# kuboyoo/alphazero-general-ori

Hardware: AMD Instinct MI355X
Metric: self-play rollouts/sec (32k boards, 2p Splendor) at 1/2/4/8 MI355X (higher is better)
Workload: dtype fp32 (network) / int8 (boards) / f64 (tree statistics)

## Files before the change

alphazero-general-ori_amd/csrc/mcts.hip:

```cpp
#include <hip/hip_runtime.h>

#include <cmath>
#include <cstring>
#include <new>

#include "../../include/splendor_amd.h"

#include "mcts_device.h"

using namespace spl;

#ifndef SPL_BOUNDS_CHECK
#define SPL_BOUNDS_CHECK 0
#endif
#if SPL_BOUNDS_CHECK
__device__ unsigned long long g_bounds[4 + 64];
__device__ __noinline__ void bounds_note(int site, long long v, int t) {
    atomicAdd(&g_bounds[4 + (site & 63)], 1ull);
    if (atomicAdd(&g_bounds[0], 1ull) == 0) {
        g_bounds[1] = (unsigned long long)v; g_bounds[2] = (unsigned long long)site; g_bounds[3] = (unsigned long long)t;
    }
}
#define BCHK(cond, site, v, t, fix)                                   \
    do {                                                               \
// ... 1730 lines not shown
    }
#endif
}

#ifndef LM_PROBE
#define LM_PROBE 0
#endif
#if LM_PROBE
constexpr int LM_PSLOTS = 4096;
__device__ unsigned long long g_lm_probe[LM_PSLOTS][8];
#define LMPROBE(k) \
    if (threadIdx.x == 0 && blockIdx.x < LM_PSLOTS) g_lm_probe[blockIdx.x][k] = __builtin_amdgcn_s_memrealtime();
#else
#define LMPROBE(k)
#endif
template <int N>
__global__ __launch_bounds__(256) void k_leaf_mask(Pools P, int B, int lim, const int8_t *__restrict__ leaf_state,
                                                   const uint8_t *__restrict__ leaf_valid,
                                                   uint64_t *__restrict__ leaf_mask,
                                                   int32_t *__restrict__ leaf_index,
                                                   int32_t *__restrict__ leaf_count) {
    using Lx = Lay<N>;
    using Cv = Conv<N>;
    constexpr int RB = 64, ST = (Lx::ROWS % 2 ? Lx::ROWS : Lx::ROWS + 1) * 8;
    __shared__ __align__(16) int8_t lds[RB * ST];
    __shared__ uint64_t mfac[7 * 116];
    __shared__ uint64_t pf0[4][RB], pf1[RB];
    __shared__ uint32_t pcond[RB];
    __shared__ uint8_t pbad[4][RB];
    __shared__ uint64_t msk[RB][7];
    LMPROBE(0)
    const int b0 = blockIdx.x * RB, nb = min(RB, B - b0);
    const int tid = threadIdx.x, w = tid >> 6, l = lane_id();
    if (w == 2 && leaf_index) {
        const bool v = l < nb && leaf_valid[b0 + l];
        const uint64_t bv = __ballot(v);
        if (v) leaf_index[b0 + __popcll(bv & lanemask_lt())] = b0 + l;
        if (l == 0) leaf_count[blockIdx.x] = __popcll(bv);
    }
    constexpr int FW = (7 * 116 + 255) / 256;
    uint64_t fw[FW];
#pragma unroll
    for (int k = 0; k < FW; k++) {
        const int i = tid + 256 * k;
        fw[k] = i < 7 * 116 ? (&K_MASK_FACTORS[0][0])[i] : 0;
    }
    if constexpr (Cv::QUAD) {
        constexpr int BU = (RB * Cv::UNITS + 255) / 256;
        uint32_t d[BU][7];
#pragma unroll
        for (int k = 0; k < BU; k++) {
            const int i = min(tid + 256 * k, nb * Cv::UNITS - 1), b = i / Cv::UNITS, u = i - b * Cv::UNITS;
            const uint32_t *g = reinterpret_cast<const uint32_t *>(leaf_state + (size_t)(b0 + b) * Lx::S) + 7 * u;
#pragma unroll
// ... 1 lines not shown
        }
#pragma unroll
        for (int k = 0; k < BU; k++) {
            const int i = tid + 256 * k, b = i / Cv::UNITS, u = i - b * Cv::UNITS;
            if (i < nb * Cv::UNITS) quad_rows_put(d[k], reinterpret_cast<uint64_t *>(lds + b * ST) + 4 * u);
        }
    } else {
        for (int i = tid; i < nb * Cv::UNITS; i += 256) {
            const int b = i / Cv::UNITS, u = i - b * Cv::UNITS;
            Cv::load(lds + b * ST, leaf_state + (size_t)(b0 + b) * Lx::S, u);
        }
    }
#pragma unroll
    for (int k = 0; k < FW; k++)
        if (tid + 256 * k < 7 * 116) mfac[tid + 256 * k] = fw[k];
    lds_sync();
    LMPROBE(1)
    if (l < nb) {
        uint64_t f0, f1;
        uint32_t cc;
        bool bad;
        const int8_t *st = lds + l * ST;
        switch (w) {
            case 0: lane_predicates_part<N, 0>(st, 0, lim, f0, f1, cc, bad); break;
            case 1: lane_predicates_part<N, 1>(st, 0, lim, f0, f1, cc, bad); break;
            case 2: lane_predicates_part<N, 2>(st, 0, lim, f0, f1, cc, bad); break;
            default: lane_predicates_part<N, 3>(st, 0, lim, f0, f1, cc, bad); break;
        }
        pf0[w][l] = f0;
        if (w == 3) pf1[l] = f1;
        if (w == 2) pcond[l] = cc;
        pbad[w][l] = bad;
// ... 26 lines not shown
        }
    }
    lds_sync();
    LMPROBE(3)
    {
        const int b = 16 * w + l;
        if (l < 16 && b < nb) {
            int cnt = 0;
#pragma unroll
            for (int k = 0; k < 7; k++) cnt += __popcll(msk[b][k]);
            if (!cnt) msk[b][6] |= 1ull << (408 - 384);
        }
    }
    lds_sync();
    LMPROBE(4)
    for (int i = tid; i < nb * 7; i += 256)
        if (leaf_valid[b0 + i / 7]) leaf_mask[(size_t)b0 * 7 + i] = (&msk[0][0])[i];
    LMPROBE(5)
}

#ifndef BK_PF
#define BK_PF 4
#endif
#ifndef BK_WIDE
#define BK_WIDE 12
#endif
#ifndef BACKUP_WAVES
#define BACKUP_WAVES 4
#endif

struct Screen {
    float L1, H1, H2, cf, ff, sqv, sqe;
// ... 1092 lines not shown
}

int spl_mcts_pick_best(spl_mcts *m, const uint8_t *active, uint32_t board_base, uint32_t stream,
                       int16_t *action, void *hs) {
    if (!m || !action || stream > 0xFFFFFFu) return SPL_EINVAL;
    hipLaunchKernelGGL(k_pick_best, wave_grid(m->B), dim3(THREADS), 0, (hipStream_t)hs, m->P, m->cfg,
                       m->B, active, board_base, stream, action);
    return check_launch();
}

static int launch_select(spl_mcts *m, int8_t *leaf_state, uint64_t *leaf_mask, uint8_t *leaf_valid,
                         int32_t *leaf_index, int32_t *leaf_count, void *hs) {
    SPL_DISPATCH(m->n, hipLaunchKernelGGL(k_select_lanes<N>, dim3((unsigned)((m->B + 63) / 64)), dim3(64), 0,
                                          (hipStream_t)hs, m->P, m->cfg, m->B, mcts_lim(m),
                                          leaf_state, leaf_valid));
    SPL_DISPATCH(m->n, hipLaunchKernelGGL(k_leaf_mask<N>, dim3((unsigned)((m->B + 63) / 64)), dim3(256), 0,
                                          (hipStream_t)hs, m->P, m->B, mcts_lim(m), leaf_state, leaf_valid,
                                          leaf_mask, leaf_index, leaf_count));
    return check_launch();
}

int spl_mcts_select(spl_mcts *m, int8_t *leaf_state, uint64_t *leaf_mask, uint8_t *leaf_valid,
                    void *hs) {
    if (!m || !leaf_state || !leaf_mask || !leaf_valid) return SPL_EINVAL;
    return launch_select(m, leaf_state, leaf_mask, leaf_valid, nullptr, nullptr, hs);
}

int spl_mcts_select_compact(spl_mcts *m, int8_t *leaf_state, uint64_t *leaf_mask, uint8_t *leaf_valid,
                            int32_t *leaf_index, int32_t *leaf_count, void *hs) {
    if (!m || !leaf_state || !leaf_mask || !leaf_valid || !leaf_index || !leaf_count) return SPL_EINVAL;
    return launch_select(m, leaf_state, leaf_mask, leaf_valid, leaf_index, leaf_count, hs);
}

int spl_mcts_backup_kind(spl_mcts *m, const uint64_t *leaf_mask, const float *pi, const float *v, int kinds,
// ... 132 lines not shown
```

alphazero-general-ori_amd/csrc/nnet.hip:

```cpp
#include <hip/hip_runtime.h>

#include "../../include/splendor_amd.h"

#ifndef NN_PROBE
#define NN_PROBE 0
#endif
#if NN_PROBE
__device__ unsigned long long g_nn_probe[16];
#define NPROBE(k)                                                  \
    if (threadIdx.x == 0) {                                        \
        const uint64_t c_ = __builtin_readcyclecounter();          \
        atomicAdd(&g_nn_probe[k], (unsigned long long)(c_ - nlast)); \
        nlast = c_;                                                \
    }
#else
#define NPROBE(k)
#endif

namespace {

typedef float f32x16 __attribute__((ext_vector_type(16)));
typedef float f32x4 __attribute__((ext_vector_type(4)));
typedef float f32x2 __attribute__((ext_vector_type(2)));

// ... 59 lines not shown
            s -= nstages(l);
        }
        return -1;
    }
    static constexpr int stg_index(int s) {
        for (int l = 0; l < 4; l++) {
            if (s < nstages(l)) return s;
            s -= nstages(l);
        }
        return -1;
    }
    static constexpr int stg_c0(int s) { return stg_index(s) ? first(stg_layer(s)) : 0; }
    static constexpr int stg_nc(int s) { return stg_index(s) ? CL[stg_layer(s)] - first(stg_layer(s)) : first(stg_layer(s)); }
};
static_assert(Net<4>::XR + RING <= BUFA, "input staging + weight ring fit bufA");

template <int V> struct IntC {
    static constexpr int value = V;
};

typedef __bf16 bf16x8 __attribute__((ext_vector_type(8)));
typedef uint32_t u32x4 __attribute__((ext_vector_type(4)));
struct F8 {
    float4 lo, hi;
};

__device__ __forceinline__ uint32_t hi_pair(uint32_t a, uint32_t b) { return __builtin_amdgcn_perm(b, a, 0x07060302u); }
__device__ __forceinline__ void split8(const F8 &x, bf16x8 &hi, bf16x8 &mid, bf16x8 &lo) {
    const float xs[8] = {x.lo.x, x.lo.y, x.lo.z, x.lo.w, x.hi.x, x.hi.y, x.hi.z, x.hi.w};
    float r1[8], r2[8];
// ... 201 lines not shown
        __builtin_amdgcn_fence(__ATOMIC_RELEASE, "wavefront");
        __builtin_amdgcn_wave_barrier();
        int f = lane < ML ? rowt[lane] : -1;
        f = max(f, __builtin_amdgcn_update_dpp(-1, f, 0x111, 0xf, 0xf, false));
        f = max(f, __builtin_amdgcn_update_dpp(-1, f, 0x112, 0xf, 0xf, false));
        f = max(f, __builtin_amdgcn_update_dpp(-1, f, 0x114, 0xf, 0xf, false));
        f = max(f, __builtin_amdgcn_update_dpp(-1, f, 0x118, 0xf, 0xf, false));
        f = max(f, __builtin_amdgcn_update_dpp(-1, f, 0x142, 0xa, 0xf, false));
        const int pos = f >= 0 ? b0 + lane + offv[f] : 0;
        __builtin_amdgcn_wave_barrier();
        if (lane < ML) rowt[lane] = pos;
    }
    return base;
}

template <int NP, int PR>
__global__ __launch_bounds__(NNT) __attribute__((amdgpu_waves_per_eu(2, 2))) void k_nn_forward(int B, const int8_t *__restrict__ state,
                                                    const uint64_t *__restrict__ mask,
                                                    const float *__restrict__ W, float *__restrict__ pi_out,
                                                    float *__restrict__ v_out,
                                                    const int32_t *__restrict__ idx,
                                                    const int32_t *__restrict__ count) {
    using Nt = Net<NP>;
    constexpr int R = Nt::R, X0S = Nt::X0S, NSTG = Nt::NSTG;
    __shared__ __align__(16) char lds[BUFA + SAB + ML * 7 * 8 + 15 * ML * 4];
    float *bufA = reinterpret_cast<float *>(lds);
    SplitAct *SB0 = reinterpret_cast<SplitAct *>(lds + BUFA);
    uint64_t *mskl = reinterpret_cast<uint64_t *>(lds + BUFA + SAB);
    const int tid = threadIdx.x, w = __builtin_amdgcn_readfirstlane(tid >> 6), lane = tid & 63, li = lane & 31;
    const int h = lane >> 5;
    const int b0 = blockIdx.x * ML;
    const float *aff = W + Nt::AFF;
    char *ring = lds + Nt::XR;
    float *biasL = reinterpret_cast<float *>(SB0);
    auto load_stage = [&](auto s_const) {
        constexpr int S = decltype(s_const)::value;
        if constexpr (S < NSTG) {
            constexpr int L = Nt::stg_layer(S), C0 = Nt::stg_c0(S), NC = Nt::stg_nc(S), C = Nt::CL[L];
            const char *src = reinterpret_cast<const char *>(W + Nt::soff(L)) + lane * 16;
            char *dst = ring + (S & 1) * RSTAGE * RSLOT;
#pragma unroll
            for (int j = 0; j < NC; j++)
#pragma unroll
                for (int b = 0; b < 4; b++)
#pragma unroll
                    for (int p = 0; p < PR; p++)
                        glds16(src + ((b * C + C0 + j) * 3 + p) * 1024, dst + ((j * 4 + b) * 3 + p) * 1024);
        }
    };
    if (w == 7) {
        load_stage(IntC<0>());
        load_stage(IntC<1>());
    }
    int *rowt = reinterpret_cast<int *>(lds + BUFA + SAB + ML * 7 * 8);
    int *rowt_w = rowt + (w < 7 ? w : 0) * ML, *rowv = rowt + 7 * ML, *offv_w = rowt + (8 + (w < 7 ? w : 0)) * ML;
    int cnt = B;
    if (count) {
        cnt = __builtin_amdgcn_readfirstlane(
            nn_list_rows(count, (B + 63) >> 6, b0, w < 7 ? rowt_w : nullptr, offv_w));
        __builtin_amdgcn_fence(__ATOMIC_RELEASE, "wavefront");
        __builtin_amdgcn_wave_barrier();
    }
    if (b0 >= cnt) {
        if (w == 7) __builtin_amdgcn_s_waitcnt(0);
        return;
    }
    const int nb = min(ML, cnt - b0);
    const auto rowin = [&](int i) -> size_t { return count ? (size_t)idx[rowt_w[i]] : (size_t)(b0 + i); };
    const auto rowof = [&](int i) -> size_t { return count ? (size_t)rowv[i] : (size_t)(b0 + i); };

#if NN_PROBE
    uint64_t nlast = __builtin_readcyclecounter();
    if (threadIdx.x == 0) atomicAdd(&g_nn_probe[15], 1ull);
#endif
    int8_t *x0 = reinterpret_cast<int8_t *>(lds);
    constexpr int NS7 = NNT - 64;
    if (w < 7) {
        if (tid < nb * 7) mskl[tid] = mask[rowin(tid / 7) * 7 + tid % 7];
        for (int t = tid; t < 4 * 128; t += NS7) {
            const int l = t >> 7, c = t & 127;
            biasL[t] = l == 2 ? (c >= 8 ? W[Nt::boff(2) + c - 8] : 0.f) : W[Nt::boff(l) + c];
        }
        if constexpr ((7 * R) % 4 == 0) {
            constexpr int BW = R * 7 / 4;
            constexpr int PER = (ML * BW + NS7 - 1) / NS7;
            int32_t d[PER];
#pragma unroll
            for (int k = 0; k < PER; k++) {
                const int j = tid + k * NS7, i = j / BW;
                d[k] = j < nb * BW ? reinterpret_cast<const int32_t *>(state + rowin(i) * R * 7)[j - i * BW] : 0;
            }
#pragma unroll
// ... 416 lines not shown
            if (i < nb) {
                const float inv = 1.f / sum[q];
#pragma unroll
                for (int k = 0; k < 7; k++) {
                    const int a = 64 * k + lane;
                    if (a < ACT) pi_out[rowof(i) * ACT + a] = x[q][k] * inv;
                }
            }
        }
    }
    NPROBE(9)
}

inline int check_launch() { return hipGetLastError() == hipSuccess ? 0 : SPL_EDEVICE; }

template <int NP>
const void *nn_kernel_np(int precision) {
    switch (precision) {
        case SPL_NN_F32: return reinterpret_cast<const void *>(&k_nn_forward<NP, 3>);
        case SPL_NN_BF16X2: return reinterpret_cast<const void *>(&k_nn_forward<NP, 2>);
        default: return reinterpret_cast<const void *>(&k_nn_forward<NP, 1>);
    }
}
inline const void *nn_kernel(int n_players, int precision) {
    switch (n_players) {
        case 2: return nn_kernel_np<2>(precision);
        case 3: return nn_kernel_np<3>(precision);
        default: return nn_kernel_np<4>(precision);
    }
}

}

extern "C" {

#if NN_PROBE
int spl_diag_nn_probe(unsigned long long *out16, int reset) {
    if (hipMemcpyFromSymbol(out16, HIP_SYMBOL(g_nn_probe), 16 * 8) != hipSuccess) return SPL_EDEVICE;
    if (reset) {
        unsigned long long z[16] = {0};
        if (hipMemcpyToSymbol(HIP_SYMBOL(g_nn_probe), z, sizeof(z)) != hipSuccess) return SPL_EDEVICE;
    }
    return 0;
// ... 4 lines not shown
    switch (n_players) {
        case 2: return Net<2>::TOTAL;
        case 3: return Net<3>::TOTAL;
        case 4: return Net<4>::TOTAL;
        default: return SPL_EINVAL;
    }
}

static int launch_nn(int n_players, int B, const int8_t *leaf_state, const uint64_t *leaf_mask,
                     const float *packed_weights, float *pi, float *v, const int32_t *idx, const int32_t *count,
                     int precision, void *hs) {
    if (n_players < 2 || n_players > 4 || B < 0 || (B && (!leaf_state || !leaf_mask || !packed_weights || !pi || !v)))
        return SPL_EINVAL;
    if (precision < SPL_NN_F32 || precision > SPL_NN_BF16) return SPL_EINVAL;
    if (!B) return 0;
    const void *kernel = nn_kernel(n_players, precision);
    void *args[] = {&B, &leaf_state, &leaf_mask, &packed_weights, &pi, &v, &idx, &count};
    if (hipLaunchKernel(kernel, dim3((unsigned)((B + ML - 1) / ML)), dim3(NNT), args, 0, (hipStream_t)hs) != hipSuccess)
        return SPL_EDEVICE;
    return check_launch();
}

int spl_nn_forward(int n_players, int B, const int8_t *leaf_state, const uint64_t *leaf_mask,
                   const float *packed_weights, float *pi, float *v, void *hs) {
    return launch_nn(n_players, B, leaf_state, leaf_mask, packed_weights, pi, v, nullptr, nullptr, SPL_NN_F32, hs);
}

int spl_nn_forward_indexed(int n_players, int B, const int8_t *leaf_state, const uint64_t *leaf_mask,
                           const int32_t *leaf_index, const int32_t *leaf_count, const float *packed_weights,
                           float *pi, float *v, void *hs) {
    if (!leaf_index || !leaf_count || reinterpret_cast<uintptr_t>(leaf_count) % 16) return SPL_EINVAL;
    return launch_nn(n_players, B, leaf_state, leaf_mask, packed_weights, pi, v, leaf_index, leaf_count, SPL_NN_F32,
                     hs);
}

int spl_nn_forward_mode(int n_players, int B, const int8_t *leaf_state, const uint64_t *leaf_mask,
                        const int32_t *leaf_index, const int32_t *leaf_count, const float *packed_weights,
                        float *pi, float *v, int precision, void *hs) {
    if (!leaf_index != !leaf_count || (leaf_count && reinterpret_cast<uintptr_t>(leaf_count) % 16)) return SPL_EINVAL;
    return launch_nn(n_players, B, leaf_state, leaf_mask, packed_weights, pi, v, leaf_index, leaf_count, precision,
                     hs);
}

}
```

alphazero-general-ori_amd/splendor/_lib.py:

```python
import ctypes as C
import os

PKG_ROOT = os.path.dirname(os.path.dirname(os.path.abspath(__file__)))
LIB_PATH = os.environ.get("SPLENDOR_AMD_LIB") or os.path.join(PKG_ROOT, "libsplendor_amd.so")

ABI_VERSION = 11
EINVAL, EDEVICE = -1, -2
ERR_BAD_ACTION, ERR_BAD_INDEX = 1, 2
BACKUP_DEFER_GC = 4
PLAYER_RANDOM, PLAYER_GREEDY, PLAYER_POLICY = 0, 1, 2
PLAYOUT_UNIFORM, PLAYOUT_BUY_FIRST = 0, 1
RULE_NO_RESERVE = 1


class NativeEngineMissing(RuntimeError):
    pass


class EngineError(RuntimeError):
    pass


_lib = None

# ... 17 lines not shown
    "spl_step": ([C.c_void_p, C.c_int, _vp, _vp, _vp, _vp, C.c_int, _vp, C.c_int, C.c_uint64,
                  C.c_uint32, C.c_uint32, _vp, _vp], C.c_int),
    "spl_game_ended": ([C.c_void_p, C.c_int, _vp, _vp, _vp], C.c_int),
    "spl_canonical": ([C.c_void_p, C.c_int, _vp, _vp, _vp, _vp], C.c_int),
    "spl_score": ([C.c_void_p, C.c_int, _vp, _vp, _vp], C.c_int),
    "spl_round": ([C.c_void_p, C.c_int, _vp, _vp, _vp], C.c_int),
    "spl_tree_step": ([C.c_void_p, C.c_int, _vp, _vp, _vp, _vp, _vp], C.c_int),
    "spl_player_move": ([C.c_void_p, C.c_int, _vp, _vp, C.c_int, _vp, C.c_uint64, C.c_uint32, C.c_uint32,
                         _vp, _vp, _vp, _vp], C.c_int),
    "spl_rollout_step": ([C.c_void_p, C.c_int, _vp, _vp, _vp, _vp, _vp, _vp, C.c_uint64, C.c_uint32,
                          C.c_uint32, _vp], C.c_int),
    "spl_nn_packed_floats": ([C.c_int], C.c_int),
    "spl_nn_forward": ([C.c_int, C.c_int, _vp, _vp, _vp, _vp, _vp, _vp], C.c_int),
    "spl_nn_forward_indexed": ([C.c_int, C.c_int, _vp, _vp, _vp, _vp, _vp, _vp, _vp, _vp], C.c_int),
    "spl_nn_forward_mode": ([C.c_int, C.c_int, _vp, _vp, _vp, _vp, _vp, _vp, _vp, C.c_int, _vp], C.c_int),
    "spl_rollout_run": ([C.c_void_p, C.c_int, C.c_int, _vp, _vp, _vp, _vp, _vp, _vp, C.c_uint64,
                         C.c_uint32, C.c_uint32, _vp], C.c_int),
    "spl_playout": ([C.c_void_p, C.c_int, _vp, _vp, _vp, C.c_int, C.c_int, C.c_int, C.c_uint64, C.c_uint32,
                     C.c_uint32, _vp, _vp, _vp, _vp, _vp], C.c_int),
    "spl_mcts_create": ([C.c_void_p, C.c_int, C.c_void_p, C.POINTER(C.c_void_p)], C.c_int),
    "spl_mcts_destroy": ([C.c_void_p], C.c_int),
    "spl_mcts_device_bytes": ([C.c_void_p], C.c_longlong),
    "spl_mcts_plan_bytes": ([_vp, C.c_int, _vp], C.c_longlong),
    "spl_mcts_counters": ([C.c_void_p, _vp, _vp], C.c_int),
    "spl_mcts_pool_state": ([C.c_void_p, _vp, _vp], C.c_int),
    "spl_mcts_pool_pages": ([C.c_void_p, _vp], C.c_int),
    "spl_mcts_set_roots": ([C.c_void_p, _vp, C.c_int, C.c_int, _vp], C.c_int),
    "spl_mcts_set_roots_active": ([C.c_void_p, _vp, _vp, C.c_int, C.c_int, _vp], C.c_int),
    "spl_mcts_pick_best": ([C.c_void_p, _vp, C.c_uint32, C.c_uint32, _vp, _vp], C.c_int),
    "spl_mcts_select": ([C.c_void_p, _vp, _vp, _vp, _vp], C.c_int),
# ... 57 lines not shown
```

alphazero-general-ori_amd/splendor/mcts.py:

```python
import ctypes as C
import os

import numpy as np
import torch

from . import _lib
from .env import ACTIONS, MASK_WORDS, _ptr

HDR_DTYPE = np.dtype([
    ("node_count", "<i4"), ("edge_count", "<i4"), ("root", "<i4"), ("sims_done", "<i4"),
    ("budget", "<i4"), ("full", "<i4"), ("noise_pending", "<i4"), ("depth", "<i4"),
    ("leaf_kind", "<i4"), ("player", "<i4"), ("episode_step", "<i4"), ("move_no", "<i4"),
    ("game_no", "<i4"), ("overflow", "<i4"), ("n_examples", "<i4"), ("leaf_round", "<i4"),
    ("leaf_k0", "<u8"), ("leaf_k1", "<u8"), ("leaf_v", "<f4", (4,)),
    ("games_done", "<i4"), ("forced", "<i4"), ("moves", "<i4"), ("wd_search", "<i4"),
    ("prunes", "<i4"), ("resets", "<i4"), ("unexpanded", "<i4"), ("gc_state", "<i4"),
    ("units_gc", "<i8"), ("enext", "<i8"),
    ("npg", "<i4"), ("epg", "<i4"), ("eleft", "<i4"), ("live_gc", "<i4"),
    ("root_round", "<i4"), ("gc_queued", "<i4"), ("withdrawals", "<i4"), ("gcs", "<i4"),
    ("leaf_hslot", "<i4"), ("leaf_slot", "<i4"), ("depth_max", "<i4"), ("depth_sum", "<i4"),
    ("resume", "<i4"), ("sims_backed", "<i4"), ("exact_wide", "<i4"), ("big_moves", "<i4")])
assert HDR_DTYPE.itemsize == 208

DEFAULT_ARGS = dict(numMCTSSims=100, cpuct=1.0, fpu=0.0, prob_fullMCTS=1.0, ratio_fullMCTS=5,
# ... 55 lines not shown
        h = C.c_void_p()
        if rules is not None:
            own = engine.rules
            engine.set_rules(flags=int(rules))
        try:
            _lib.check(self.L.spl_mcts_create(engine.ctx, B, C.byref(cfg), C.byref(h)), "spl_mcts_create")
        finally:
            if rules is not None:
                engine.set_rules(flags=own)
        self.h = h
        dev = engine.device
        self.leaf_state = engine.new_state(B)
        self.leaf_mask = torch.zeros((B, MASK_WORDS), dtype=torch.int64, device=dev)
        self.leaf_valid = torch.zeros(B, dtype=torch.uint8, device=dev)
        self.leaf_index = torch.zeros(B, dtype=torch.int32, device=dev)
        self.leaf_count = torch.zeros((B + 63) // 64, dtype=torch.int32, device=dev)
        self.evaluator = evaluator or HashEvaluator(engine)
        self._hdr = torch.empty((B, HDR_DTYPE.itemsize // 4), dtype=torch.int32, device=dev)

    MEM_FRACTION = 0.8
    UNITS_PER_NODE = 20
    NODE_MAX = 45056

    @staticmethod
    def default_node_cap(sims):
        return min(64 * sims + 4096, BatchedMCTS.NODE_MAX)

    def _plan(self, engine, B, sims, cfg, node_cap, edge_cap, pool_nodes, pool_edges, auto_boards, mem_budget):
        nc = int(node_cap or self.default_node_cap(sims))
        ec = int(edge_cap or 32 * nc)
        cfg.node_cap, cfg.edge_cap = nc, ec
        cfg.pool_nodes, cfg.pool_edges = int(pool_nodes or 0), int(pool_edges or 0)
# ... 62 lines not shown
    def set_roots(self, roots, keep_tree=True, force_full=True):
        _lib.check(self.L.spl_mcts_set_roots(self.h, _ptr(roots), int(keep_tree), int(force_full),
                                             self.e._s()), "spl_mcts_set_roots")

    def set_roots_active(self, roots, active, keep_tree=True, force_full=True):
        _lib.check(self.L.spl_mcts_set_roots_active(self.h, _ptr(roots), _ptr(active), int(keep_tree),
                                                    int(force_full), self.e._s()),
                   "spl_mcts_set_roots_active")

    def pick_best(self, active=None, board_base=0, stream=0, out=None):
        out = out if out is not None else torch.full((self.B,), -1, dtype=torch.int16, device=self.e.device)
        _lib.check(self.L.spl_mcts_pick_best(self.h, _ptr(active), int(board_base), int(stream), _ptr(out),
                                             self.e._s()), "spl_mcts_pick_best")
        return out

    def search(self):
        for _ in range(int(self.headers()["budget"].max())):
            self.simulate()

    OVERLAP_TERMINAL = os.environ.get("SPLENDOR_OVERLAP", "0") != "0"

    def simulate(self, defer_gc=False):
        s = self.e._s()
        dg = _lib.BACKUP_DEFER_GC if defer_gc else 0
        if getattr(self.evaluator, "indexed", False):
            _lib.check(self.L.spl_mcts_select_compact(self.h, _ptr(self.leaf_state), _ptr(self.leaf_mask),
                                                      _ptr(self.leaf_valid), _ptr(self.leaf_index),
                                                      _ptr(self.leaf_count), s), "spl_mcts_select_compact")
            if self.OVERLAP_TERMINAL and self.e.device.type == "cuda":
                cur = torch.cuda.current_stream(self.e.device)
                side = getattr(self, "_side", None)
                if side is None:
                    side = self._side = torch.cuda.Stream(device=self.e.device)
                side.wait_stream(cur)
                _lib.check(self.L.spl_mcts_backup_kind(self.h, None, None, None, 2, C.c_void_p(side.cuda_stream)),
                           "spl_mcts_backup_kind")
                pi, v = self.evaluator(self.leaf_state, self.leaf_mask, self.leaf_valid, index=self.leaf_index,
                                       count=self.leaf_count)
                cur.wait_stream(side)
                _lib.check(self.L.spl_mcts_backup_kind(self.h, _ptr(self.leaf_mask), _ptr(pi), _ptr(v), 1 | dg, s),
                           "spl_mcts_backup_kind")
                return
            pi, v = self.evaluator(self.leaf_state, self.leaf_mask, self.leaf_valid, index=self.leaf_index,
                                   count=self.leaf_count)
        else:
            _lib.check(self.L.spl_mcts_select(self.h, _ptr(self.leaf_state), _ptr(self.leaf_mask),
                                              _ptr(self.leaf_valid), s), "spl_mcts_select")
            pi, v = self.evaluator(self.leaf_state, self.leaf_mask, self.leaf_valid)
        _lib.check(self.L.spl_mcts_backup_kind(self.h, _ptr(self.leaf_mask), _ptr(pi), _ptr(v), 3 | dg, s),
                   "spl_mcts_backup_kind")

    def headers(self):
        _lib.check(self.L.spl_mcts_headers(self.h, _ptr(self._hdr), self.e._s()), "spl_mcts_headers")
        return self._hdr.cpu().numpy().view(HDR_DTYPE).reshape(self.B)

    def tree_sizes(self):
        out = torch.empty((self.B, 4), dtype=torch.int32, device=self.e.device)
        _lib.check(self.L.spl_mcts_tree_sizes(self.h, _ptr(out), self.e._s()), "spl_mcts_tree_sizes")
        return out.cpu().numpy()
# ... 39 lines not shown
```

alphazero-general-ori_amd/splendor/nnet.py:

```python
import ctypes as C

import torch
import torch.nn as nn
import torch.nn.functional as F

from . import _lib
from .env import ACTIONS, _ptr


def _lin(i, o):
    m = nn.Linear(i, o)
    nn.init.kaiming_uniform_(m.weight)
    nn.init.zeros_(m.bias)
    return m


class _PoolDense(nn.Module):

    def __init__(self, width, groups, items, bn_channels):
        super().__init__()
        self.groups, self.items = groups, items
        self.dense_part = nn.Sequential(_lin(width - groups * items, width - 2 * groups),
                                        nn.BatchNorm1d(bn_channels))

# ... 241 lines not shown
    pi = lin(lin(x, f.wpi1, f.bpi1), f.wpi2, f.bpi2).double()
    pi = torch.softmax(pi.masked_fill(~valid, -1e8), 1)
    v = torch.tanh(lin(lin(x, f.wv1, f.bv1), f.wv2, f.bv2).double())
    return pi, v


class FusedNet:

    def __init__(self, net, n_players, device, precision="f32"):
        self.n = n_players
        self.device = torch.device(device)
        self.precision = precision
        self.mode = precision_mode(precision)
        self.w = pack_weights(FoldedNet(net).to(self.device).eval(), n_players)

    def __call__(self, leaf_state, leaf_mask, pi=None, v=None, index=None, count=None):
        B = leaf_state.shape[0]
        pi = pi if pi is not None else torch.empty((B, ACTIONS), dtype=torch.float32, device=self.device)
        v = v if v is not None else torch.empty((B, self.n), dtype=torch.float32, device=self.device)
        s = C.c_void_p(torch.cuda.current_stream(self.device).cuda_stream)
        if self.mode:
            _lib.check(_lib.lib().spl_nn_forward_mode(self.n, B, _ptr(leaf_state), _ptr(leaf_mask), _ptr(index),
                                                      _ptr(count), _ptr(self.w), _ptr(pi), _ptr(v), self.mode, s),
                       "spl_nn_forward_mode")
        elif index is None:
            _lib.check(_lib.lib().spl_nn_forward(self.n, B, _ptr(leaf_state), _ptr(leaf_mask), _ptr(self.w),
                                                 _ptr(pi), _ptr(v), s), "spl_nn_forward")
        else:
            _lib.check(_lib.lib().spl_nn_forward_indexed(self.n, B, _ptr(leaf_state), _ptr(leaf_mask), _ptr(index),
                                                         _ptr(count), _ptr(self.w), _ptr(pi), _ptr(v), s),
                       "spl_nn_forward_indexed")
        return pi, v


def random_net(n_players=2, seed=0, device="cuda"):
    g = torch.random.fork_rng(devices=[])
    with g:
        torch.manual_seed(seed)
        net = SplendorNNet(n_players)
    return net.to(device).eval()


class LeafEvaluator:

    def __init__(self, engine, net, B, use_graph=True, fused=True, precision="f32"):
        self.e = engine
        self.B = B
# ... 15 lines not shown

    def _convert(self, leaf_state, leaf_mask):
        _lib.check(self.e.L.spl_nn_input(self.e.ctx, self.B, _ptr(leaf_state), _ptr(leaf_mask),
                                         _ptr(self.x), C.c_void_p(self.valid.data_ptr()), self.e._s()),
                   "spl_nn_input")

    @torch.no_grad()
    def _run(self, leaf_state, leaf_mask):
        self._convert(leaf_state, leaf_mask)
        return self.net(self.x, self.valid, transposed=True)

    @property
    def indexed(self):
        return self.fused is not None

    @torch.no_grad()
    def __call__(self, leaf_state, leaf_mask, leaf_valid=None, index=None, count=None):
        if self.fused is not None:
            return self.fused(leaf_state, leaf_mask, self.pi_buf, self.v_buf, index=index, count=count)
        if not self.use_graph:
            return self._run(leaf_state, leaf_mask)
        key = (leaf_state.data_ptr(), leaf_mask.data_ptr())
        if self.graph is None or key != (self._state_ptr, self._mask_ptr):
            s = torch.cuda.Stream(self.e.device)
            s.wait_stream(torch.cuda.current_stream(self.e.device))
            with torch.cuda.stream(s):
                for _ in range(2):
                    self._run(leaf_state, leaf_mask)
            torch.cuda.current_stream(self.e.device).wait_stream(s)
            self.graph = torch.cuda.CUDAGraph()
            with torch.cuda.graph(self.graph):
                self.pi, self.v = self._run(leaf_state, leaf_mask)
            self._state_ptr, self._mask_ptr = key
        self.graph.replay()
# ... 2 lines not shown
```

include/splendor_amd.h:

```cpp
#ifndef SPLENDOR_AMD_H
#define SPLENDOR_AMD_H
#include <stdint.h>
#ifdef __cplusplus
extern "C" {
#endif

#define SPL_ABI_VERSION 11
#define SPL_ACTIONS 409
#define SPL_MASK_WORDS 7
#define SPL_EINVAL (-1)
#define SPL_EDEVICE (-2)
#define SPL_ERR_BAD_ACTION 1
#define SPL_ERR_BAD_INDEX 2

typedef struct spl_ctx spl_ctx;

int spl_abi_version(void);

int spl_ctx_create(int n_players, int token_limit, spl_ctx **out);
int spl_ctx_destroy(spl_ctx *ctx);
int spl_ctx_set_token_limit(spl_ctx *ctx, int token_limit);
#define SPL_RULE_NO_RESERVE 1
int spl_ctx_set_rules(spl_ctx *ctx, int flags);
int spl_ctx_rules(const spl_ctx *ctx);
// ... 133 lines not shown

int spl_nn_packed_floats(int n_players);
int spl_nn_forward(int n_players, int B, const int8_t *leaf_state, const uint64_t *leaf_mask,
                   const float *packed_weights, float *pi, float *v, void *hip_stream);
int spl_nn_forward_indexed(int n_players, int B, const int8_t *leaf_state, const uint64_t *leaf_mask,
                           const int32_t *leaf_index, const int32_t *leaf_count, const float *packed_weights,
                           float *pi, float *v, void *hip_stream);
#define SPL_NN_F32 0
#define SPL_NN_BF16X2 1
#define SPL_NN_BF16 2
int spl_nn_forward_mode(int n_players, int B, const int8_t *leaf_state, const uint64_t *leaf_mask,
                        const int32_t *leaf_index, const int32_t *leaf_count,
                        const float *packed_weights, float *pi, float *v, int precision,
                        void *hip_stream);

#ifdef __cplusplus
}
#endif
#endif
```

Measured before the change: 73.67 million.

## Stage compacted, pre-transposed leaf tiles for the NN forward in leaf-mask kernel

The leaf-mask kernel now computes a global prefix count of valid leaves and writes the valid leaves densely into a staging buffer. Each leaf's board rows are written already transposed into the NN kernel's 32-row tile layout, along with compacted masks and a row map. The NN forward gets a staged variant that copies whole tile images straight into LDS with 16-byte loads instead of doing per-row gathers and index-list reconstruction. This moves layout work into a kernel that already holds the data in LDS. In exchange, every leaf-mask block re-reads all preceding valid flags to compute its prefix, which grows quadratically with grid size, and the staging memory adds write traffic.

Measured after the change: 75.28 million (median of 6 runs). 1.02x the previous value.

```diff
diff --git a/alphazero-general-ori_amd/csrc/mcts.hip b/alphazero-general-ori_amd/csrc/mcts.hip
--- a/alphazero-general-ori_amd/csrc/mcts.hip
+++ b/alphazero-general-ori_amd/csrc/mcts.hip
@@ -7,6 +7,7 @@
 #include "../../include/splendor_amd.h"
 
 #include "mcts_device.h"
+#include "nn_stage.h"
 
 using namespace spl;
 
@@ -1768,21 +1769,29 @@
 #else
 #define LMPROBE(k)
 #endif
-template <int N>
+__device__ __forceinline__ int nonzero_bytes(uint32_t x) {
+    return __popc((((x & 0x7F7F7F7Fu) + 0x7F7F7F7Fu) | x) & 0x80808080u);
+}
+template <int N, bool STG = false>
 __global__ __launch_bounds__(256) void k_leaf_mask(Pools P, int B, int lim, const int8_t *__restrict__ leaf_state,
                                                    const uint8_t *__restrict__ leaf_valid,
                                                    uint64_t *__restrict__ leaf_mask,
                                                    int32_t *__restrict__ leaf_index,
-                                                   int32_t *__restrict__ leaf_count) {
+                                                   int32_t *__restrict__ leaf_count,
+                                                   char *__restrict__ stage) {
     using Lx = Lay<N>;
     using Cv = Conv<N>;
     constexpr int RB = 64, ST = (Lx::ROWS % 2 ? Lx::ROWS : Lx::ROWS + 1) * 8;
+    static_assert(Lx::ROWS == nnstage::rows(N) && 4 * ((Lx::ROWS + 3) / 4) <= nnstage::x0s(N) &&
+                      nnstage::TILE == 32, "staged tile image (nn_stage.h)");
     __shared__ __align__(16) int8_t lds[RB * ST];
     __shared__ uint64_t mfac[7 * 116];
     __shared__ uint64_t pf0[4][RB], pf1[RB];
     __shared__ uint32_t pcond[RB];
     __shared__ uint8_t pbad[4][RB];
     __shared__ uint64_t msk[RB][7];
+    __shared__ int wsum[4];
+    __shared__ int8_t lst[STG ? RB : 1], rnk[STG ? RB : 1];
     LMPROBE(0)
     const int b0 = blockIdx.x * RB, nb = min(RB, B - b0);
     const int tid = threadIdx.x, w = tid >> 6, l = lane_id();
@@ -1792,6 +1801,25 @@
         if (v) leaf_index[b0 + __popcll(bv & lanemask_lt())] = b0 + l;
         if (l == 0) leaf_count[blockIdx.x] = __popcll(bv);
     }
+    int pre = 0, rank = 0, nlist = 0;
+    bool vme = false;
+    if constexpr (STG) {
+        constexpr int VB = 8;
+        const int nu = blockIdx.x * 4;
+        const uint4 *vv = reinterpret_cast<const uint4 *>(leaf_valid);
+        for (int u0 = 0; u0 < nu; u0 += 256 * VB) {
+            uint4 q[VB];
+#pragma unroll
+            for (int k = 0; k < VB; k++) {
+                const int u = u0 + 256 * k + tid;
+                q[k] = u < nu ? vv[u] : uint4{0u, 0u, 0u, 0u};
+            }
+#pragma unroll
+            for (int k = 0; k < VB; k++)
+                pre += nonzero_bytes(q[k].x) + nonzero_bytes(q[k].y) + nonzero_bytes(q[k].z) + nonzero_bytes(q[k].w);
+        }
+        vme = l < nb && leaf_valid[b0 + l];
+    }
     constexpr int FW = (7 * 116 + 255) / 256;
     uint64_t fw[FW];
 #pragma unroll
@@ -1823,8 +1851,63 @@
 #pragma unroll
     for (int k = 0; k < FW; k++)
         if (tid + 256 * k < 7 * 116) mfac[tid + 256 * k] = fw[k];
+    if constexpr (STG) {
+#pragma unroll
+        for (int o = 32; o > 0; o >>= 1) pre += __shfl_xor(pre, o, 64);
+        const uint64_t bv = __ballot(vme);
+        rank = __popcll(bv & lanemask_lt());
+        nlist = __popcll(bv);
+        if (w == 0) {
+            if (l == 0) wsum[0] = pre;
+            if (vme) lst[rank] = (int8_t)l;
+            rnk[l] = vme ? (int8_t)rank : (int8_t)-1;
+        } else if (l == 0) {
+            wsum[w] = pre;
+        }
+    }
     lds_sync();
     LMPROBE(1)
+    int base = 0;
+    if constexpr (STG) {
+        base = (wsum[0] + wsum[1]) + (wsum[2] + wsum[3]);
+        constexpr int G = (Lx::ROWS + 3) / 4, X0S = nnstage::x0s(N), TB = nnstage::tile_bytes(N);
+        char *sx = stage + nnstage::x_off(B);
+        for (int it = tid; it < nlist * G; it += 256) {
+            const int q = it / G, g = it - q * G, p = base + q;
+            const uint64_t *rw = reinterpret_cast<const uint64_t *>(lds + lst[q] * ST) + 4 * g;
+            uint32_t lo[4], hi[4];
+#pragma unroll
+            for (int j = 0; j < 4; j++) {
+                const uint64_t a = 4 * g + j < Lx::ROWS ? rw[j] : 0ull;
+                lo[j] = (uint32_t)a;
+                hi[j] = (uint32_t)(a >> 32);
+            }
+            uint32_t col[7];
+            {
+                const uint32_t t01 = __builtin_amdgcn_perm(lo[1], lo[0], 0x05010400u), t23 = __builtin_amdgcn_perm(lo[3], lo[2], 0x05010400u);
+                const uint32_t u01 = __builtin_amdgcn_perm(lo[1], lo[0], 0x07030602u), u23 = __builtin_amdgcn_perm(lo[3], lo[2], 0x07030602u);
+                col[0] = __builtin_amdgcn_perm(t23, t01, 0x05040100u);
+                col[1] = __builtin_amdgcn_perm(t23, t01, 0x07060302u);
+                col[2] = __builtin_amdgcn_perm(u23, u01, 0x05040100u);
+                col[3] = __builtin_amdgcn_perm(u23, u01, 0x07060302u);
+            }
+            {
+                const uint32_t t01 = __builtin_amdgcn_perm(hi[1], hi[0], 0x05010400u), t23 = __builtin_amdgcn_perm(hi[3], hi[2], 0x05010400u);
+                const uint32_t u01 = __builtin_amdgcn_perm(hi[1], hi[0], 0x07030602u), u23 = __builtin_amdgcn_perm(hi[3], hi[2], 0x07030602u);
+                col[4] = __builtin_amdgcn_perm(t23, t01, 0x05040100u);
+                col[5] = __builtin_amdgcn_perm(t23, t01, 0x07060302u);
+                col[6] = __builtin_amdgcn_perm(u23, u01, 0x05040100u);
+            }
+            if (p < B) {
+                uint32_t *dst = reinterpret_cast<uint32_t *>(sx + (size_t)(p >> 5) * TB + (p & 31) * X0S) + g;
+#pragma unroll
+                for (int c = 0; c < 7; c++) dst[c * (32 * X0S / 4)] = col[c];
+            }
+        }
+        if (w == 0 && vme && base + rank < B)
+            reinterpret_cast<int32_t *>(stage + nnstage::ROWS_OFF)[base + rank] = b0 + l;
+        if (blockIdx.x == gridDim.x - 1 && tid == 0) *reinterpret_cast<int32_t *>(stage) = base + nlist;
+    }
     if (l < nb) {
         uint64_t f0, f1;
         uint32_t cc;
@@ -1881,8 +1964,20 @@
     }
     lds_sync();
     LMPROBE(4)
-    for (int i = tid; i < nb * 7; i += 256)
-        if (leaf_valid[b0 + i / 7]) leaf_mask[(size_t)b0 * 7 + i] = (&msk[0][0])[i];
+    if constexpr (STG) {
+        uint64_t *smask = reinterpret_cast<uint64_t *>(stage + nnstage::mask_off(B));
+        for (int i = tid; i < nb * 7; i += 256) {
+            const int lf = i / 7, r = rnk[lf];
+            if (r >= 0) {
+                const uint64_t mw = (&msk[0][0])[i];
+                leaf_mask[(size_t)b0 * 7 + i] = mw;
+                if (base + r < B) smask[(size_t)(base + r) * 7 + (i - 7 * lf)] = mw;
+            }
+        }
+    } else {
+        for (int i = tid; i < nb * 7; i += 256)
+            if (leaf_valid[b0 + i / 7]) leaf_mask[(size_t)b0 * 7 + i] = (&msk[0][0])[i];
+    }
     LMPROBE(5)
 }
 
@@ -3005,10 +3100,44 @@
     SPL_DISPATCH(m->n, hipLaunchKernelGGL(k_select_lanes<N>, dim3((unsigned)((m->B + 63) / 64)), dim3(64), 0,
                                           (hipStream_t)hs, m->P, m->cfg, m->B, mcts_lim(m),
                                           leaf_state, leaf_valid));
+    char *no_stage = nullptr;
     SPL_DISPATCH(m->n, hipLaunchKernelGGL(k_leaf_mask<N>, dim3((unsigned)((m->B + 63) / 64)), dim3(256), 0,
                                           (hipStream_t)hs, m->P, m->B, mcts_lim(m), leaf_state, leaf_valid,
-                                          leaf_mask, leaf_index, leaf_count));
+                                          leaf_mask, leaf_index, leaf_count, no_stage));
     return check_launch();
+}
+
+static int launch_mask_staged(int n, const Pools &P, int B, int lim, const int8_t *leaf_state,
+                              const uint8_t *leaf_valid, uint64_t *leaf_mask, void *stage, void *hs) {
+    int32_t *no_list = nullptr;
+    char *st = static_cast<char *>(stage);
+    SPL_DISPATCH(n, hipLaunchKernelGGL((k_leaf_mask<N, true>), dim3((unsigned)((B + 63) / 64)), dim3(256), 0,
+                                       (hipStream_t)hs, P, B, lim, leaf_state, leaf_valid, leaf_mask, no_list,
+                                       no_list, st));
+    return check_launch();
+}
+static bool stage_args_ok(const void *leaf_state, const void *leaf_mask, const void *leaf_valid, const void *stage) {
+    return leaf_state && leaf_mask && leaf_valid && stage && reinterpret_cast<uintptr_t>(leaf_state) % 4 == 0 &&
+           reinterpret_cast<uintptr_t>(leaf_mask) % 8 == 0 && reinterpret_cast<uintptr_t>(leaf_valid) % 16 == 0 &&
+           reinterpret_cast<uintptr_t>(stage) % 16 == 0;
+}
+
+int spl_mcts_select_staged(spl_mcts *m, int8_t *leaf_state, uint64_t *leaf_mask, uint8_t *leaf_valid, void *stage,
+                           void *hs) {
+    if (!m || !stage_args_ok(leaf_state, leaf_mask, leaf_valid, stage)) return SPL_EINVAL;
+    SPL_DISPATCH(m->n, hipLaunchKernelGGL(k_select_lanes<N>, dim3((unsigned)((m->B + 63) / 64)), dim3(64), 0,
+                                          (hipStream_t)hs, m->P, m->cfg, m->B, mcts_lim(m),
+                                          leaf_state, leaf_valid));
+    return launch_mask_staged(m->n, m->P, m->B, mcts_lim(m), leaf_state, leaf_valid, leaf_mask, stage, hs);
+}
+
+int spl_nn_stage_leaves(const spl_ctx *ctx, int B, const int8_t *leaf_state, const uint8_t *leaf_valid,
+                        uint64_t *leaf_mask, void *stage, void *hs) {
+    if (!ctx || ctx->n < 2 || ctx->n > 4 || B < 0 || !stage_args_ok(leaf_state, leaf_mask, leaf_valid, stage))
+        return SPL_EINVAL;
+    if (!B) return 0;
+    return launch_mask_staged(ctx->n, Pools{}, B, pack_lim(ctx->token_limit, ctx->rules), leaf_state, leaf_valid,
+                              leaf_mask, stage, hs);
 }
 
 int spl_mcts_select(spl_mcts *m, int8_t *leaf_state, uint64_t *leaf_mask, uint8_t *leaf_valid,
diff --git a/alphazero-general-ori_amd/csrc/nn_stage.h b/alphazero-general-ori_amd/csrc/nn_stage.h
--- /dev/null
+++ b/alphazero-general-ori_amd/csrc/nn_stage.h
@@ -0,0 +1,22 @@
+#pragma once
+#include <cstddef>
+
+namespace nnstage {
+
+constexpr int TILE = 32;
+__host__ __device__ constexpr int rows(int np) { return 32 + 10 * np + np * np; }
+__host__ __device__ constexpr int x0s(int np) {
+    const int kp = (rows(np) + 7) / 8 * 8;
+    return (kp / 4) % 2 ? kp : kp + 4;
+}
+__host__ __device__ constexpr int tile_bytes(int np) { return 7 * TILE * x0s(np); }
+__host__ __device__ constexpr size_t align16(size_t x) { return (x + 15) / 16 * 16; }
+constexpr size_t ROWS_OFF = 16;
+__host__ __device__ constexpr size_t mask_off(int B) { return align16(ROWS_OFF + 4 * (size_t)B); }
+__host__ __device__ constexpr size_t x_off(int B) { return align16(mask_off(B) + 56 * (size_t)B); }
+__host__ __device__ constexpr size_t bytes(int np, int B) {
+    return x_off(B) + (size_t)((B + TILE - 1) / TILE) * tile_bytes(np);
+}
+static_assert(tile_bytes(2) % 16 == 0 && tile_bytes(3) % 16 == 0 && tile_bytes(4) % 16 == 0, "16-byte tile copies");
+
+}
diff --git a/alphazero-general-ori_amd/csrc/nnet.hip b/alphazero-general-ori_amd/csrc/nnet.hip
--- a/alphazero-general-ori_amd/csrc/nnet.hip
+++ b/alphazero-general-ori_amd/csrc/nnet.hip
@@ -1,6 +1,7 @@
 #include <hip/hip_runtime.h>
 
 #include "../../include/splendor_amd.h"
+#include "nn_stage.h"
 
 #ifndef NN_PROBE
 #define NN_PROBE 0
@@ -97,6 +98,12 @@
     static constexpr int stg_nc(int s) { return stg_index(s) ? CL[stg_layer(s)] - first(stg_layer(s)) : first(stg_layer(s)); }
 };
 static_assert(Net<4>::XR + RING <= BUFA, "input staging + weight ring fit bufA");
+static_assert(ML == nnstage::TILE, "staged tiles are this kernel's tiles");
+static_assert(Net<2>::R == nnstage::rows(2) && Net<3>::R == nnstage::rows(3) && Net<4>::R == nnstage::rows(4), "board rows");
+static_assert(Net<2>::X0S == nnstage::x0s(2) && Net<3>::X0S == nnstage::x0s(3) && Net<4>::X0S == nnstage::x0s(4),
+              "staged image stride");
+static_assert(Net<2>::XR == nnstage::tile_bytes(2) && Net<3>::XR == nnstage::tile_bytes(3) &&
+                  Net<4>::XR == nnstage::tile_bytes(4), "a staged tile is the whole input image");
 
 template <int V> struct IntC {
     static constexpr int value = V;
@@ -328,13 +335,14 @@
     return base;
 }
 
-template <int NP, int PR>
+template <int NP, int PR, bool STG = false>
 __global__ __launch_bounds__(NNT) __attribute__((amdgpu_waves_per_eu(2, 2))) void k_nn_forward(int B, const int8_t *__restrict__ state,
                                                     const uint64_t *__restrict__ mask,
                                                     const float *__restrict__ W, float *__restrict__ pi_out,
                                                     float *__restrict__ v_out,
                                                     const int32_t *__restrict__ idx,
-                                                    const int32_t *__restrict__ count) {
+                                                    const int32_t *__restrict__ count,
+                                                    const char *__restrict__ sbuf) {
     using Nt = Net<NP>;
     constexpr int R = Nt::R, X0S = Nt::X0S, NSTG = Nt::NSTG;
     __shared__ __align__(16) char lds[BUFA + SAB + ML * 7 * 8 + 15 * ML * 4];
@@ -362,6 +370,8 @@
                         glds16(src + ((b * C + C0 + j) * 3 + p) * 1024, dst + ((j * 4 + b) * 3 + p) * 1024);
         }
     };
+    int scnt = 0;
+    if constexpr (STG) scnt = *reinterpret_cast<const int32_t *>(sbuf);
     if (w == 7) {
         load_stage(IntC<0>());
         load_stage(IntC<1>());
@@ -369,7 +379,9 @@
     int *rowt = reinterpret_cast<int *>(lds + BUFA + SAB + ML * 7 * 8);
     int *rowt_w = rowt + (w < 7 ? w : 0) * ML, *rowv = rowt + 7 * ML, *offv_w = rowt + (8 + (w < 7 ? w : 0)) * ML;
     int cnt = B;
-    if (count) {
+    if constexpr (STG) {
+        cnt = min(__builtin_amdgcn_readfirstlane(scnt), B);
+    } else if (count) {
         cnt = __builtin_amdgcn_readfirstlane(
             nn_list_rows(count, (B + 63) >> 6, b0, w < 7 ? rowt_w : nullptr, offv_w));
         __builtin_amdgcn_fence(__ATOMIC_RELEASE, "wavefront");
@@ -381,7 +393,7 @@
     }
     const int nb = min(ML, cnt - b0);
     const auto rowin = [&](int i) -> size_t { return count ? (size_t)idx[rowt_w[i]] : (size_t)(b0 + i); };
-    const auto rowof = [&](int i) -> size_t { return count ? (size_t)rowv[i] : (size_t)(b0 + i); };
+    const auto rowof = [&](int i) -> size_t { return STG || count ? (size_t)rowv[i] : (size_t)(b0 + i); };
 
 #if NN_PROBE
     uint64_t nlast = __builtin_readcyclecounter();
@@ -389,7 +401,38 @@
 #endif
     int8_t *x0 = reinterpret_cast<int8_t *>(lds);
     constexpr int NS7 = NNT - 64;
-    if (w < 7) {
+    if constexpr (STG) {
+        if (w < 7) {
+            constexpr int UN = 7 * ML * X0S / 16, PER = (UN + NS7 - 1) / NS7;
+            const u32x4 *src = reinterpret_cast<const u32x4 *>(sbuf + nnstage::x_off(B)) + (size_t)blockIdx.x * UN;
+            const uint64_t *smask = reinterpret_cast<const uint64_t *>(sbuf + nnstage::mask_off(B)) + (size_t)b0 * 7;
+            const int32_t *srows = reinterpret_cast<const int32_t *>(sbuf + nnstage::ROWS_OFF) + b0;
+            const u32x4 d0 = src[min(tid, UN - 1)], d1 = src[min(tid + NS7, UN - 1)];
+            const u32x4 d2 = PER > 2 ? src[min(tid + 2 * NS7, UN - 1)] : d1;
+            static_assert(PER <= 3, "tile image: at most three 16-byte units per thread");
+            const uint64_t mk = smask[min(tid, nb * 7 - 1)];
+            const int rw = srows[min(lane, nb - 1)];
+            static_assert(4 * 128 <= 2 * NS7, "per-column biases: two per thread");
+            const int t1 = min(tid + NS7, 4 * 128 - 1);
+            const auto bias_of = [&](int t) {
+                const int l = t >> 7, c = t & 127;
+                return l == 2 ? (c >= 8 ? W[Nt::boff(2) + c - 8] : 0.f) : W[Nt::boff(l) + c];
+            };
+            const float bl0 = bias_of(tid), bl1 = bias_of(t1);
+            u32x4 *xl = reinterpret_cast<u32x4 *>(lds);
+            if (tid < UN) xl[tid] = d0;
+            if (tid + NS7 < UN) xl[tid + NS7] = d1;
+            if (PER > 2 && tid + 2 * NS7 < UN) xl[tid + 2 * NS7] = d2;
+            if (tid < nb * 7) mskl[tid] = mk;
+            if (w == 0 && lane < nb) rowv[lane] = rw;
+            biasL[tid] = bl0;
+            if (tid + NS7 < 4 * 128) biasL[tid + NS7] = bl1;
+        } else {
+            constexpr int N1 = 4 * PR * Nt::stg_nc(1);
+            static_assert(N1 < 64, "vmcnt range");
+            __builtin_amdgcn_s_waitcnt((N1 & 15) | ((N1 >> 4) << 14) | (7 << 4) | (15 << 8));
+        }
+    } else if (w < 7) {
         if (tid < nb * 7) mskl[tid] = mask[rowin(tid / 7) * 7 + tid % 7];
         for (int t = tid; t < 4 * 128; t += NS7) {
             const int l = t >> 7, c = t & 127;
@@ -836,19 +879,20 @@
 
 inline int check_launch() { return hipGetLastError() == hipSuccess ? 0 : SPL_EDEVICE; }
 
-template <int NP>
+template <int NP, bool STG>
 const void *nn_kernel_np(int precision) {
     switch (precision) {
-        case SPL_NN_F32: return reinterpret_cast<const void *>(&k_nn_forward<NP, 3>);
-        case SPL_NN_BF16X2: return reinterpret_cast<const void *>(&k_nn_forward<NP, 2>);
-        default: return reinterpret_cast<const void *>(&k_nn_forward<NP, 1>);
-    }
-}
-inline const void *nn_kernel(int n_players, int precision) {
+        case SPL_NN_F32: return reinterpret_cast<const void *>(&k_nn_forward<NP, 3, STG>);
+        case SPL_NN_BF16X2: return reinterpret_cast<const void *>(&k_nn_forward<NP, 2, STG>);
+        default: return reinterpret_cast<const void *>(&k_nn_forward<NP, 1, STG>);
+    }
+}
+template <bool STG>
+const void *nn_kernel(int n_players, int precision) {
     switch (n_players) {
-        case 2: return nn_kernel_np<2>(precision);
-        case 3: return nn_kernel_np<3>(precision);
-        default: return nn_kernel_np<4>(precision);
+        case 2: return nn_kernel_np<2, STG>(precision);
+        case 3: return nn_kernel_np<3, STG>(precision);
+        default: return nn_kernel_np<4, STG>(precision);
     }
 }
 
@@ -883,8 +927,9 @@
         return SPL_EINVAL;
     if (precision < SPL_NN_F32 || precision > SPL_NN_BF16) return SPL_EINVAL;
     if (!B) return 0;
-    const void *kernel = nn_kernel(n_players, precision);
-    void *args[] = {&B, &leaf_state, &leaf_mask, &packed_weights, &pi, &v, &idx, &count};
+    const void *kernel = nn_kernel<false>(n_players, precision);
+    const char *stage = nullptr;
+    void *args[] = {&B, &leaf_state, &leaf_mask, &packed_weights, &pi, &v, &idx, &count, &stage};
     if (hipLaunchKernel(kernel, dim3((unsigned)((B + ML - 1) / ML)), dim3(NNT), args, 0, (hipStream_t)hs) != hipSuccess)
         return SPL_EDEVICE;
     return check_launch();
@@ -911,4 +956,26 @@
                      hs);
 }
 
-}
+long long spl_nn_stage_bytes(int n_players, int B) {
+    if (n_players < 2 || n_players > 4 || B < 0) return SPL_EINVAL;
+    return (long long)nnstage::bytes(n_players, B);
+}
+
+int spl_nn_forward_staged(int n_players, int B, const void *stage, const float *packed_weights, float *pi, float *v,
+                          int precision, void *hs) {
+    if (n_players < 2 || n_players > 4 || B < 0 || !stage || !packed_weights || !pi || !v) return SPL_EINVAL;
+    if (reinterpret_cast<uintptr_t>(stage) % 16 || reinterpret_cast<uintptr_t>(packed_weights) % 16) return SPL_EINVAL;
+    if (precision < SPL_NN_F32 || precision > SPL_NN_BF16) return SPL_EINVAL;
+    if (!B) return 0;
+    const void *kernel = nn_kernel<true>(n_players, precision);
+    const int8_t *no_state = nullptr;
+    const uint64_t *no_mask = nullptr;
+    const int32_t *no_list = nullptr;
+    const char *st = static_cast<const char *>(stage);
+    void *args[] = {&B, &no_state, &no_mask, &packed_weights, &pi, &v, &no_list, &no_list, &st};
+    if (hipLaunchKernel(kernel, dim3((unsigned)((B + ML - 1) / ML)), dim3(NNT), args, 0, (hipStream_t)hs) != hipSuccess)
+        return SPL_EDEVICE;
+    return check_launch();
+}
+
+}
diff --git a/alphazero-general-ori_amd/splendor/_lib.py b/alphazero-general-ori_amd/splendor/_lib.py
--- a/alphazero-general-ori_amd/splendor/_lib.py
+++ b/alphazero-general-ori_amd/splendor/_lib.py
@@ -55,6 +55,10 @@
     "spl_nn_forward": ([C.c_int, C.c_int, _vp, _vp, _vp, _vp, _vp, _vp], C.c_int),
     "spl_nn_forward_indexed": ([C.c_int, C.c_int, _vp, _vp, _vp, _vp, _vp, _vp, _vp, _vp], C.c_int),
     "spl_nn_forward_mode": ([C.c_int, C.c_int, _vp, _vp, _vp, _vp, _vp, _vp, _vp, C.c_int, _vp], C.c_int),
+    "spl_nn_stage_bytes": ([C.c_int, C.c_int], C.c_longlong),
+    "spl_nn_stage_leaves": ([C.c_void_p, C.c_int, _vp, _vp, _vp, _vp, _vp], C.c_int),
+    "spl_nn_forward_staged": ([C.c_int, C.c_int, _vp, _vp, _vp, _vp, C.c_int, _vp], C.c_int),
+    "spl_mcts_select_staged": ([C.c_void_p, _vp, _vp, _vp, _vp, _vp], C.c_int),
     "spl_rollout_run": ([C.c_void_p, C.c_int, C.c_int, _vp, _vp, _vp, _vp, _vp, _vp, C.c_uint64,
                          C.c_uint32, C.c_uint32, _vp], C.c_int),
     "spl_playout": ([C.c_void_p, C.c_int, _vp, _vp, _vp, C.c_int, C.c_int, C.c_int, C.c_uint64, C.c_uint32,
diff --git a/alphazero-general-ori_amd/splendor/mcts.py b/alphazero-general-ori_amd/splendor/mcts.py
--- a/alphazero-general-ori_amd/splendor/mcts.py
+++ b/alphazero-general-ori_amd/splendor/mcts.py
@@ -93,8 +93,10 @@
         self.leaf_mask = torch.zeros((B, MASK_WORDS), dtype=torch.int64, device=dev)
         self.leaf_valid = torch.zeros(B, dtype=torch.uint8, device=dev)
         self.leaf_index = torch.zeros(B, dtype=torch.int32, device=dev)
-        self.leaf_count = torch.zeros((B + 63) // 64, dtype=torch.int32, device=dev)
+        self._leaf_count = torch.zeros((B + 63) // 64, dtype=torch.int32, device=dev)
         self.evaluator = evaluator or HashEvaluator(engine)
+        self.stage = None
+        self._staged_select = False
         self._hdr = torch.empty((B, HDR_DTYPE.itemsize // 4), dtype=torch.int32, device=dev)
 
     MEM_FRACTION = 0.8
@@ -187,6 +189,20 @@
                                              self.e._s()), "spl_mcts_pick_best")
         return out
 
+    NN_STAGED = os.environ.get("SPLENDOR_NN_STAGED", "1") != "0"
+
+    @property
+    def leaf_count(self):
+        return self.stage[:4].view(torch.int32) if self._staged_select else self._leaf_count
+
+    def _stage_buf(self):
+        if not (self.NN_STAGED and getattr(self.evaluator, "staged", False)):
+            return None
+        if self.stage is None:
+            from .nnet import new_stage
+            self.stage = new_stage(self.e.n, self.B, self.e.device)
+        return self.stage
+
     def search(self):
         for _ in range(int(self.headers()["budget"].max())):
             self.simulate()
@@ -196,10 +212,19 @@
     def simulate(self, defer_gc=False):
         s = self.e._s()
         dg = _lib.BACKUP_DEFER_GC if defer_gc else 0
-        if getattr(self.evaluator, "indexed", False):
-            _lib.check(self.L.spl_mcts_select_compact(self.h, _ptr(self.leaf_state), _ptr(self.leaf_mask),
-                                                      _ptr(self.leaf_valid), _ptr(self.leaf_index),
-                                                      _ptr(self.leaf_count), s), "spl_mcts_select_compact")
+        stage = self._stage_buf()
+        self._staged_select = stage is not None
+        if stage is not None or getattr(self.evaluator, "indexed", False):
+            if stage is not None:
+                _lib.check(self.L.spl_mcts_select_staged(self.h, _ptr(self.leaf_state), _ptr(self.leaf_mask),
+                                                         _ptr(self.leaf_valid), _ptr(stage), s),
+                           "spl_mcts_select_staged")
+                how = dict(stage=stage)
+            else:
+                _lib.check(self.L.spl_mcts_select_compact(self.h, _ptr(self.leaf_state), _ptr(self.leaf_mask),
+                                                          _ptr(self.leaf_valid), _ptr(self.leaf_index),
+                                                          _ptr(self._leaf_count), s), "spl_mcts_select_compact")
+                how = dict(index=self.leaf_index, count=self._leaf_count)
             if self.OVERLAP_TERMINAL and self.e.device.type == "cuda":
                 cur = torch.cuda.current_stream(self.e.device)
                 side = getattr(self, "_side", None)
@@ -208,14 +233,12 @@
                 side.wait_stream(cur)
                 _lib.check(self.L.spl_mcts_backup_kind(self.h, None, None, None, 2, C.c_void_p(side.cuda_stream)),
                            "spl_mcts_backup_kind")
-                pi, v = self.evaluator(self.leaf_state, self.leaf_mask, self.leaf_valid, index=self.leaf_index,
-                                       count=self.leaf_count)
+                pi, v = self.evaluator(self.leaf_state, self.leaf_mask, self.leaf_valid, **how)
                 cur.wait_stream(side)
                 _lib.check(self.L.spl_mcts_backup_kind(self.h, _ptr(self.leaf_mask), _ptr(pi), _ptr(v), 1 | dg, s),
                            "spl_mcts_backup_kind")
                 return
-            pi, v = self.evaluator(self.leaf_state, self.leaf_mask, self.leaf_valid, index=self.leaf_index,
-                                   count=self.leaf_count)
+            pi, v = self.evaluator(self.leaf_state, self.leaf_mask, self.leaf_valid, **how)
         else:
             _lib.check(self.L.spl_mcts_select(self.h, _ptr(self.leaf_state), _ptr(self.leaf_mask),
                                               _ptr(self.leaf_valid), s), "spl_mcts_select")
diff --git a/alphazero-general-ori_amd/splendor/nnet.py b/alphazero-general-ori_amd/splendor/nnet.py
--- a/alphazero-general-ori_amd/splendor/nnet.py
+++ b/alphazero-general-ori_amd/splendor/nnet.py
@@ -279,12 +279,17 @@
         self.mode = precision_mode(precision)
         self.w = pack_weights(FoldedNet(net).to(self.device).eval(), n_players)
 
-    def __call__(self, leaf_state, leaf_mask, pi=None, v=None, index=None, count=None):
+    staged = True
+
+    def __call__(self, leaf_state, leaf_mask, pi=None, v=None, index=None, count=None, stage=None):
         B = leaf_state.shape[0]
         pi = pi if pi is not None else torch.empty((B, ACTIONS), dtype=torch.float32, device=self.device)
         v = v if v is not None else torch.empty((B, self.n), dtype=torch.float32, device=self.device)
         s = C.c_void_p(torch.cuda.current_stream(self.device).cuda_stream)
-        if self.mode:
+        if stage is not None:
+            _lib.check(_lib.lib().spl_nn_forward_staged(self.n, B, _ptr(stage), _ptr(self.w), _ptr(pi), _ptr(v),
+                                                        self.mode, s), "spl_nn_forward_staged")
+        elif self.mode:
             _lib.check(_lib.lib().spl_nn_forward_mode(self.n, B, _ptr(leaf_state), _ptr(leaf_mask), _ptr(index),
                                                       _ptr(count), _ptr(self.w), _ptr(pi), _ptr(v), self.mode, s),
                        "spl_nn_forward_mode")
@@ -296,6 +301,13 @@
                                                          _ptr(count), _ptr(self.w), _ptr(pi), _ptr(v), s),
                        "spl_nn_forward_indexed")
         return pi, v
+
+
+def new_stage(n_players, B, device):
+    nbytes = int(_lib.lib().spl_nn_stage_bytes(n_players, B))
+    if nbytes < 0:
+        raise _lib.EngineError(f"spl_nn_stage_bytes({n_players}, {B}): invalid argument")
+    return torch.zeros(nbytes, dtype=torch.uint8, device=device)
 
 
 def random_net(n_players=2, seed=0, device="cuda"):
@@ -341,10 +353,14 @@
     def indexed(self):
         return self.fused is not None
 
+    @property
+    def staged(self):
+        return self.fused is not None and self.indexed
+
     @torch.no_grad()
-    def __call__(self, leaf_state, leaf_mask, leaf_valid=None, index=None, count=None):
+    def __call__(self, leaf_state, leaf_mask, leaf_valid=None, index=None, count=None, stage=None):
         if self.fused is not None:
-            return self.fused(leaf_state, leaf_mask, self.pi_buf, self.v_buf, index=index, count=count)
+            return self.fused(leaf_state, leaf_mask, self.pi_buf, self.v_buf, index=index, count=count, stage=stage)
         if not self.use_graph:
             return self._run(leaf_state, leaf_mask)
         key = (leaf_state.data_ptr(), leaf_mask.data_ptr())
diff --git a/include/splendor_amd.h b/include/splendor_amd.h
--- a/include/splendor_amd.h
+++ b/include/splendor_amd.h
@@ -171,6 +171,14 @@
                         const float *packed_weights, float *pi, float *v, int precision,
                         void *hip_stream);
 
+long long spl_nn_stage_bytes(int n_players, int B);
+int spl_mcts_select_staged(spl_mcts *m, int8_t *leaf_state, uint64_t *leaf_mask, uint8_t *leaf_valid,
+                           void *stage, void *hip_stream);
+int spl_nn_stage_leaves(const spl_ctx *ctx, int B, const int8_t *leaf_state, const uint8_t *leaf_valid,
+                        uint64_t *leaf_mask, void *stage, void *hip_stream);
+int spl_nn_forward_staged(int n_players, int B, const void *stage, const float *packed_weights,
+                          float *pi, float *v, int precision, void *hip_stream);
+
 #ifdef __cplusplus
 }
 #endif
```
